# 123456jack/decision-making-and-path-planning

Hardware: AMD Instinct MI355X
Metric: planning ticks/sec (batched scenes), 512x512 grid (higher is better)
Workload: dtype f64; 1 GPU; BASELINE configs[1]: 1024 scenes/GPU, 512x512 grid, 64 static obstacles; scenes_per_gpu=1024, global_scenes=1024, grid=512, obstacles=64, parallelism=scene-sharded x1, RCCL scatter/gather outside the timed region, algorithmic_bytes_per_tick=276644

## Files before the change

### decision-making-and-path-planning_amd/csrc/kernels_s.hpp

```cpp
#pragma once
#include <type_traits>
#include "dev_geom.hpp"

#ifndef DMPP_PRIO_T2
#define DMPP_PRIO_T2 12
#define DMPP_PRIO_T3 36
#endif
namespace dmpp {

__device__ __forceinline__ uint64_t mix64(uint64_t v)
{
    uint64_t z = v + 0x9e3779b97f4a7c15ull;
    z = (z ^ (z >> 30)) * 0xbf58476d1ce4e5b9ull;
    z = (z ^ (z >> 27)) * 0x94d049bb133111ebull;
    return z ^ (z >> 31);
}

__device__ __forceinline__ int cell_of(const PlannerConfig& c, GlobalPoint2D origin, double x, double y)
{
    int ix = (int)floor((x - origin.x) / c.cell);
    int iy = (int)floor((y - origin.y) / c.cell);
    ix = clampi(ix, 0, c.grid_w - 1); iy = clampi(iy, 0, c.grid_h - 1);
    return iy * c.grid_w + ix;
}
// ... 169 lines not shown
            run = (go && stop != 0u && !((B0 >> bit) & 1u)) ? (int)((uint32_t)rr | (fP << 12) | (fM << 13)) : run;
            go = go && stop == 0u && cand != 0;
        }
    }
    return run;
}

struct Footprint { double ox, oy, R2; int ix0, ix1, iy0, iy1; };

__device__ __forceinline__ Footprint footprint_of(const PlannerConfig& c, GlobalPoint2D origin, const ObPoint& o, int W, int H)
{
    Footprint f;
    const double R = (double)o.radius + c.inflate;
    f.ox = o.x; f.oy = o.y; f.R2 = R * R;
    f.ix0 = max((int)floor((o.x - R - origin.x) / c.cell) - 1, 0);
    f.ix1 = min((int)floor((o.x + R - origin.x) / c.cell) + 1, W - 1);
    f.iy0 = max((int)floor((o.y - R - origin.y) / c.cell) - 1, 0);
    f.iy1 = min((int)floor((o.y + R - origin.y) / c.cell) + 1, H - 1);
    return f;
}

__device__ __forceinline__ bool exact_span(double ou, double org, double cell, double inv_cell, double dv2, double R2, double cq, int ic,
                                           int lo, int hi, int& a, int& b)
{
    if (dv2 > R2) return false;
    auto pred = [&](int i) { const double du = (org + ((double)i + 0.5) * cell) - ou; return du * du + dv2 <= R2; };
    const double h2 = R2 - dv2;
    const double half = __builtin_amdgcn_sqrt(h2);
    const double xa = (ou - half - org) * inv_cell - 0.5, xb = (ou + half - org) * inv_cell - 0.5;
    a = clampi((int)ceil(xa), lo - 1, hi + 1);
    b = clampi((int)floor(xb), lo - 1, hi + 1);
    {
        const double lim = 0.5 - (half * 0x1p-24 + cq) * inv_cell;
        const bool sure = (h2 >= R2 * 0x1p-40) & (fabs((xa - floor(xa)) - 0.5) < lim) & (fabs((xb - floor(xb)) - 0.5) < lim);
        if (__builtin_expect(sure, 1)) { a = max(a, lo); b = min(b, hi); return a <= b; }
    }
    asm volatile("" : "+v"(ic), "+v"(lo), "+v"(hi));
    const bool pa = pred(a), pa1 = pred(a - 1), pb = pred(b), pb1 = pred(b + 1);
    if (__builtin_expect(!((a <= b) & pa & !pa1 & pb & !pb1), 0)) {
        const bool c0 = pred(ic), c1 = pred(ic - 1), c2 = pred(ic + 1);
        if (!(c0 | c1 | c2)) return false;
        const int t = c0 ? ic : (c1 ? ic - 1 : ic + 1);
        if ((t < lo && !pred(lo)) || (t > hi && !pred(hi))) return false;
        a = clampi(min(a, t), lo - 1, hi + 1); b = clampi(max(b, t), lo - 1, hi + 1);
#pragma nounroll
        while (a >= lo && pred(a - 1)) a--;
#pragma nounroll
        while (a <= hi && !pred(a)) a++;
#pragma nounroll
        while (b <= hi && pred(b + 1)) b++;
#pragma nounroll
        while (b >= lo && b >= a && !pred(b)) b--;
    }
    a = max(a, lo); b = min(b, hi);
    return a <= b;
}

template <class F>
__device__ __forceinline__ void for_words(int p0, int p1, F&& f)
{
    for (int w = p0 >> 5; w <= (p1 >> 5); w++) {
        const int lo = max(p0 - (w << 5), 0), hi = min(p1 - (w << 5), 31);
        const uint32_t bits = (hi == 31 ? 0xFFFFFFFFu : ((2u << hi) - 1u)) & ~((1u << lo) - 1u);
        f(w, bits);
    }
}

template <int SW>
__device__ __forceinline__ int block_excl_scan(int v, int tid, int* s_wave )
{
    const int lane = tid & 63, wv = tid >> 6;
    int incl = v;
#pragma unroll
    for (int sft = 1; sft < DMPP_WAVE; sft <<= 1) { const int t = __shfl_up(incl, sft, 64); if (lane >= sft) incl += t; }
    if (lane == DMPP_WAVE - 1) s_wave[wv] = incl;
    __syncthreads();
    int base = 0, total = 0;
    for (int q = 0; q < SW; q++) { const int t = s_wave[q]; if (q < wv) base += t; total += t; }
    if (tid == 0) s_wave[SW] = total;
    __syncthreads();
    return base + incl - v;
}

template <int SW, class Emit>
__device__ __forceinline__ void for_each_span(const PlannerConfig& c, const SceneIn& si, const ObPoint* __restrict__ obs, int m, Emit&& emit)
{
    const int tid = threadIdx.x, lane = tid & 63, wv = tid >> 6;
    const int W = c.grid_w, H = c.grid_h;
    const bool colhalf = lane >= 32;
    const int l32 = lane & 31;
    const double cell = c.cell, inv_cell = 1.0 / c.cell;
    const GlobalPoint2D origin = si.grid_origin;
    const double org_u = colhalf ? origin.y : origin.x, org_v = colhalf ? origin.x : origin.y;
    const double cq_scene = 0x1p-47 * (2.0 * (fabs(origin.x) + fabs(origin.y)) + (double)max(W, H) * cell) + 0x1p-36 * cell;
    auto bcast_d = [](double v, int src) {
        const int lo = __builtin_amdgcn_readlane(__double2loint(v), src), hi = __builtin_amdgcn_readlane(__double2hiint(v), src);
        return __hiloint2double(hi, lo);
    };
    for (int base = 0; base < m; base += SW * DMPP_WAVE) {
        Footprint f; f.ox = f.oy = f.R2 = 0; f.ix0 = f.iy0 = 0; f.ix1 = f.iy1 = -1;
        int icx = 0, icy = 0;
        const int j = base + wv + SW * lane;
        if (j < m) {
            f = footprint_of(c, origin, obs[j], W, H);
            icx = (int)floor((f.ox - origin.x) / cell);
            icy = (int)floor((f.oy - origin.y) / cell);
        }
        const unsigned long long anym = wave_ballot(j < m && f.ix1 >= f.ix0 && f.iy1 >= f.iy0);
        const int left = m - base - wv;
        const int cnt = left <= 0 ? 0 : min(DMPP_WAVE, (left + SW - 1) / SW);
        for (int q = 0; q < cnt; q++) {
            if (!((anym >> q) & 1ull)) continue;
            const double fx = bcast_d(f.ox, q), fy = bcast_d(f.oy, q), R2 = bcast_d(f.R2, q);
            const int ix0 = __builtin_amdgcn_readlane(f.ix0, q), ix1 = __builtin_amdgcn_readlane(f.ix1, q);
            const int iy0 = __builtin_amdgcn_readlane(f.iy0, q), iy1 = __builtin_amdgcn_readlane(f.iy1, q);
            const int jcx = __builtin_amdgcn_readlane(icx, q), jcy = __builtin_amdgcn_readlane(icy, q);
            const double ou = colhalf ? fy : fx, ov = colhalf ? fx : fy;
            const int ic = colhalf ? jcy : jcx, l0 = colhalf ? ix0 : iy0, l1 = colhalf ? ix1 : iy1, lo = colhalf ? iy0 : ix0, hi = colhalf ? iy1 : ix1;
            const double cq = cq_scene + 0x1p-30 * (1.0 + R2);
            for (int l = l0 + l32; l <= l1; l += 32) {
                const double dv = (org_v + ((double)l + 0.5) * cell) - ov;
                int a, b;
                const bool any = exact_span(ou, org_u, cell, inv_cell, dv * dv, R2, cq, ic, lo, hi, a, b);
                if (any) emit(colhalf, l, a, b);
            }
        }
    }
}

template <int SW, class Emit>
__device__ __forceinline__ void for_each_rough_span(const PlannerConfig& c, const SceneIn& si, const ObPoint* __restrict__ obs, int m, Emit&& emit)
{
    const int tid = threadIdx.x, lane = tid & 63, wv = tid >> 6;
    const int W = c.grid_w, H = c.grid_h;
    const bool colhalf = lane >= 32;
    const int l32 = lane & 31;
    const float cellf = (float)c.cell, inv_cellf = (float)(1.0 / c.cell);
    const GlobalPoint2D origin = si.grid_origin;
    const double extent = (double)max(W, H) * c.cell;
    auto bcast_f = [](float v, int src) { return __int_as_float(__builtin_amdgcn_readlane(__float_as_int(v), src)); };
    for (int base = 0; base < m; base += SW * DMPP_WAVE) {
        float rx = 0, ry = 0, r2m = -1.0f;
        int ix0 = 0, ix1 = -1, iy0 = 0, iy1 = -1;
        const int j = base + wv + SW * lane;
        if (j < m) {
            const Footprint f = footprint_of(c, origin, obs[j], W, H);
            ix0 = f.ix0; ix1 = f.ix1; iy0 = f.iy0; iy1 = f.iy1;
            const double R = sqrt(f.R2), S = extent + R;
            rx = (float)(f.ox - origin.x); ry = (float)(f.oy - origin.y);
            r2m = (float)((f.R2 + 4.0 * (R * S * 0x1p-21 + f.R2 * 0x1p-23)) * (1.0 + 0x1p-22));
        }
        const unsigned long long anym = wave_ballot(j < m && ix1 >= ix0 && iy1 >= iy0);
        const int left = m - base - wv;
        const int cnt = left <= 0 ? 0 : min(DMPP_WAVE, (left + SW - 1) / SW);
        for (int q = 0; q < cnt; q++) {
            if (!((anym >> q) & 1ull)) continue;
            const float fx = bcast_f(rx, q), fy = bcast_f(ry, q), R2 = bcast_f(r2m, q);
            const int jx0 = __builtin_amdgcn_readlane(ix0, q), jx1 = __builtin_amdgcn_readlane(ix1, q);
            const int jy0 = __builtin_amdgcn_readlane(iy0, q), jy1 = __builtin_amdgcn_readlane(iy1, q);
            const float ou = colhalf ? fy : fx, ov = colhalf ? fx : fy;
            const int l0 = colhalf ? jx0 : jy0, l1 = colhalf ? jx1 : jy1, lo = colhalf ? jy0 : jx0, hi = colhalf ? jy1 : jx1;
            for (int l = l0 + l32; l <= l1; l += 32) {
                const float dv = ((float)l + 0.5f) * cellf - ov;
                const float h2 = R2 - dv * dv;
                if (h2 < 0.0f) continue;
                const float half = __builtin_sqrtf(h2);
                const int a = max((int)floorf((ou - half) * inv_cellf) - 2, lo), b = min((int)floorf((ou + half) * inv_cellf) + 2, hi);
                if (a <= b) emit(colhalf, l, a, b);
            }
        }
    }
}

template <int K, int SW>
__device__ __forceinline__ int build_sparse_views(const PlannerConfig& c, const SceneIn& si, const ObPoint* __restrict__ obs, int m,
                                                  const SparseView<K>& vr, const SparseView<K>& vc, int budget, int* s_wave,
                                                  long long* tmark = nullptr)
{
    using M = typename SparseView<K>::M;
    const int tid = threadIdx.x;
    const int W = c.grid_w, H = c.grid_h;
    int tm_i = 0;
    auto mark = [&]() { if (tmark) tmark[tm_i++] = clock64(); };
    mark();
    for (int l = tid; l < H; l += (SW * DMPP_WAVE)) vr.clear_line(l);
    for (int l = tid; l < W; l += (SW * DMPP_WAVE)) vc.clear_line(l);
    __syncthreads();
    mark(); mark();
    auto mark_words = [&](bool colhalf, int l, int a, int b) {
        const int wa = a >> 5, wb = b >> 5;
        const M bits = (M)((((M)2) << (wb - wa)) - (M)1) << wa;
        if (colhalf) vc.or_mask(l, bits); else vr.or_mask(l, bits);
    };
#ifdef DMPP_EXACT_PASS1
    for_each_span<SW>(c, si, obs, m, mark_words);
#else
    for_each_rough_span<SW>(c, si, obs, m, mark_words);
#endif
    __syncthreads();
    mark();
    auto place = [&](const SparseView<K>& vw) {
        const int NL = vw.NL, per = (NL + (SW * DMPP_WAVE) - 1) / (SW * DMPP_WAVE);
        const int l0 = tid * per, l1 = min(l0 + per, NL);
        int cnt = 0;
        for (int l = l0; l < l1; l++) cnt += popc_m(vw.mask_of(l));
        int off = block_excl_scan<SW>(cnt, tid, s_wave);
        const int total = s_wave[SW];
        for (int l = l0; l < l1; l++) { const int k = popc_m(vw.mask_of(l)); vw.set_off(l, (uint32_t)off); off += k; }
        __syncthreads();
        return total;
    };
    const int total_r = place(vr), total_c = place(vc);
    const int need = max(total_r, total_c);
    mark();
    if (need > budget) return need;
    for (int i = tid; i < total_r; i += (SW * DMPP_WAVE)) vr.data[i] = 0;
    for (int i = tid; i < total_c; i += (SW * DMPP_WAVE)) vc.data[i] = 0;
    __syncthreads();
    mark();
    const SparseView<K> vw = (tid & 32) ? vc : vr;
    for_each_span<SW>(c, si, obs, m, [&](bool, int l, int a, int b) {
        const LineM<M> lm = vw.line(l);
        for_words(a, b, [&](int w, uint32_t bits) {
            __hip_atomic_fetch_or(&vw.data[lm.off + popc_m((M)(lm.mask & ((((M)1) << w) - (M)1)))], bits, __ATOMIC_RELAXED, __HIP_MEMORY_SCOPE_WORKGROUP);
        });
    });
    __syncthreads();
    mark();
    return need;
}

template <int SW>
__device__ __forceinline__ void build_dense_views(const PlannerConfig& c, const SceneIn& si, const ObPoint* __restrict__ obs, int m,
                                                  uint32_t* __restrict__ bm, DMPP_LDS uint64_t* nz_row, DMPP_LDS uint64_t* nz_col)
{
    const int tid = threadIdx.x;
    const int W = c.grid_w, H = c.grid_h, WW = W >> 5, HW = H >> 5, NW = (W * H) >> 5;
    uint32_t* bmT = bm + NW;
    {
        uint4* z4 = reinterpret_cast<uint4*>(bm);
        const uint4 z = { 0u, 0u, 0u, 0u };
        for (int i = tid; i < (2 * NW) >> 2; i += (SW * DMPP_WAVE)) z4[i] = z;
    }
    __threadfence();
    __syncthreads();
    for_each_span<SW>(c, si, obs, m, [&](bool colhalf, int l, int a, int b) {
        uint32_t* line = colhalf ? bmT + (size_t)l * HW : bm + (size_t)l * WW;
        for_words(a, b, [&](int w, uint32_t bits) { atomicOr(&line[w], bits); });
    });
    __threadfence();
    __syncthreads();
    for (int v = 0; v < 2; v++) {
        const uint32_t* src = v ? bmT : bm;
        DMPP_LDS uint64_t* nz = v ? nz_col : nz_row;
        const int LW = v ? HW : WW, NL = v ? W : H;
        for (int line = tid; line < NL; line += (SW * DMPP_WAVE)) {
            uint64_t msk = 0;
            for (int w = 0; w < LW; w++) msk |= (uint64_t)min(src[line * LW + w], 1u) << w;
            nz[line] = msk;
        }
    }
    __syncthreads();
}

template <int K>
__device__ __forceinline__ void sparse_clear_cell(const SparseView<K>& vw, int line, int pos)
{
    using M = typename SparseView<K>::M;
    const LineM<M> lm = vw.line(line);
    const int w = pos >> 5;
    if (lm.mask & (((M)1) << w)) vw.data[lm.off + popc_m((M)(lm.mask & ((((M)1) << w) - (M)1)))] &= ~(1u << (pos & 31));
}

namespace rules {
constexpr int dxs(int s) { return (s == 0 || s == 1 || s == 7) ? 1 : ((s >= 3 && s <= 5) ? -1 : 0); }
constexpr int dys(int s) { return (s >= 1 && s <= 3) ? 1 : ((s >= 5) ? -1 : 0); }
constexpr int rule_code(int d, int s)
{
    const int rel = (s - d) & 7;
    const bool is_start = d == 8, d_odd = (d & 1) != 0 && !is_start, d_even = !d_odd && !is_start;
    const bool jump0 = (is_start && (s & 1) == 0) || (d_even && rel == 0) || (d_odd && (rel == 1 || rel == 7));
    const bool plain = (is_start && (s & 1) != 0) || (d_odd && rel == 0);
    const bool sided = (d_even && (rel == 1 || rel == 7)) || (d_odd && (rel == 2 || rel == 6));
    return jump0 ? 1 : (plain ? 2 : (sided ? 3 : 0));
}
constexpr int side_offset(int d, int s, bool want_y)
{
    const bool d_odd = (d & 1) != 0 && d != 8;
    const int a = want_y ? dys(s) - dys(d & 7) : dxs(s) - dxs(d & 7);
    return d_odd ? a / 2 : a;
}
constexpr uint64_t code_rows(int d0)
{
    uint64_t t = 0;
    for (int d = d0; d < d0 + 4; d++) for (int s = 0; s < 8; s++) t |= (uint64_t)rule_code(d, s) << ((d - d0) * 16 + 2 * s);
    return t;
}
constexpr uint32_t start_row() { uint32_t t = 0; for (int s = 0; s < 8; s++) t |= (uint32_t)rule_code(8, s) << (2 * s); return t; }
constexpr uint32_t kDxTab = 0x901Au, kDyTab = 0x01A9u;
constexpr bool tables_ok()
{
    for (int d = 0; d < 8; d++) if (((int)((kDxTab >> (2 * d)) & 3u) - 1) != dxs(d) || ((int)((kDyTab >> (2 * d)) & 3u) - 1) != dys(d)) return false;
    for (int d = 0; d <= 8; d++) for (int s = 0; s < 8; s++) if (rule_code(d, s) == 3) {
        const int ax = dxs(s) - dxs(d & 7), ay = dys(s) - dys(d & 7);
        if ((ax >> (d & 1)) != side_offset(d, s, false) || (ay >> (d & 1)) != side_offset(d, s, true)) return false;
    }
    return true;
}
static_assert(tables_ok(), "direction tables / side offsets");
constexpr uint64_t kCodeLo = code_rows(0), kCodeHi = code_rows(4);
constexpr uint32_t kCodeStart = start_row();
}

template <int CL>
struct SearchLds {
    static constexpr int kClosedLog = CL, kClosedTab = 1 << CL, kClosedMax = 3 << (CL - 2);
    uint32_t o_ent[kOpenCap];
    uint16_t o_f2[kOpenCap];
    uint16_t o_run[kOpenCap];
    uint32_t c_tab[kClosedTab];
    uint16_t c_info[kClosedTab];
    uint16_t c_seq[kClosedTab];
    uint32_t job[kMaxDiag + 8];
    int s_wave[kSearchSetupWavesWide + 1];
    int s_flag;
};

struct SearchOut { int status, n_exp, n_push, n_rounds, path_cost, path_len; uint64_t digest; };

template <class LDS>
__device__ __forceinline__ uint64_t hash_digest(const LDS& L, int lane)
{
    uint64_t dg = 0;
    for (int i = lane; i < LDS::kClosedTab; i += DMPP_WAVE) {
        const uint32_t e = L.c_tab[i]; const uint32_t sq = L.c_seq[i];
        if (e && sq != 0xFFFFu) dg += mix64(((uint64_t)sq << 32) | (uint64_t)(e - 1u));
    }
    return dg;
}

template <class LDS>
__device__ __forceinline__ int squeeze_open(LDS& L, int n_open, int lane)
{
    int w = 0;
    for (int q0 = 0; q0 < n_open; q0 += DMPP_WAVE) {
        const int i = q0 + lane;
        uint32_t f2 = 0xFFFFu, ee = 0; uint16_t rr = 0;
        if (i < n_open) { f2 = L.o_f2[i]; ee = L.o_ent[i]; rr = L.o_run[i]; }
        const bool alive = f2 != 0xFFFFu;
        const unsigned long long am = wave_ballot(alive);
        wave_order();
        if (alive) {
            const int r = (int)__builtin_amdgcn_mbcnt_hi((unsigned)(am >> 32), __builtin_amdgcn_mbcnt_lo((unsigned)am, 0u));
            L.o_f2[w + r] = (uint16_t)f2; L.o_ent[w + r] = ee; L.o_run[w + r] = rr;
        }
        w += __popcll(am);
        wave_order();
    }
    for (int i = w + lane; i < n_open; i += DMPP_WAVE) L.o_f2[i] = 0xFFFFu;
    wave_order();
    return w;
}

template <class LDS>
__device__ __forceinline__ int spill_open(LDS& L, int n_open , int lane, uint2* __restrict__ ospill, int& sp_n, uint32_t& sp_min)
{
    constexpr int keep = kOpenCap / 2;
    if (n_open <= keep) return n_open;
    uint32_t K[kOpenCap / DMPP_WAVE];
#pragma unroll
    for (int k = 0; k < kOpenCap / DMPP_WAVE; k++) {
        const int slot = lane + DMPP_WAVE * k;
        K[k] = slot < n_open ? (((uint32_t)L.o_f2[slot] << 16) | (0xFFFFu - (uint32_t)slot)) : 0xFFFFFFFFu;
    }
    uint32_t lo = 0u, hi = 0xFFFFFFFEu;
    for (int it = 0; it < 32 && lo < hi; it++) {
        const uint32_t mid = lo + ((hi - lo) >> 1);
        int cnt = 0;
#pragma unroll
        for (int k = 0; k < kOpenCap / DMPP_WAVE; k++) cnt += __popcll(wave_ballot(K[k] <= mid));
        if (cnt >= keep) hi = mid; else lo = mid + 1u;
    }
    uint32_t mn = 0xFFFFu;
    int base = sp_n;
#pragma unroll
    for (int k = 0; k < kOpenCap / DMPP_WAVE; k++) {
        const int slot = lane + DMPP_WAVE * k;
        const bool out = slot < n_open && K[k] > lo;
        const unsigned long long bm = wave_ballot(out);
        if (out) {
            const int r = (int)__builtin_amdgcn_mbcnt_hi((unsigned)(bm >> 32), __builtin_amdgcn_mbcnt_lo((unsigned)bm, 0u));
            const uint32_t f2 = L.o_f2[slot];
            ospill[base + r] = make_uint2(L.o_ent[slot], f2 | ((uint32_t)L.o_run[slot] << 16));
            L.o_f2[slot] = 0xFFFFu;
            mn = min(mn, f2);
        }
        base += __popcll(bm);
    }
    sp_n = base;
    sp_min = min(sp_min, wave_min_u32(mn));
// ... 461 lines not shown
            wave_sync();
            for (int i = lane; i < keep / 2; i += DMPP_WAVE) {
                const int a0 = path[i], b0 = path[keep - 1 - i];
                path[i] = b0; path[keep - 1 - i] = a0;
            }
        }
    }
    DBG_MARK(6)
    int n_push = my_pushes;
#pragma unroll
    for (int sft = 32; sft >= 1; sft >>= 1) n_push += __shfl_xor(n_push, sft, 64);
    n_push += 1;
    R.status = status; R.n_exp = n_exp; R.n_push = n_push; R.n_rounds = n_rounds; R.path_cost = path_cost; R.path_len = path_len; R.digest = digest;
    return R;
#undef DBG_MARK
}

template <class LDS>
__device__ __forceinline__ void reset_search_lds(LDS& L, int start, int goal, int W, int lane)
{
    for (int i = lane; i < LDS::kClosedTab; i += DMPP_WAVE) L.c_tab[i] = 0;
    for (int i = lane; i < kOpenCap; i += DMPP_WAVE) L.o_f2[i] = 0xFFFFu;
    wave_order();
    if (lane == 0) {
        const int sx = start % W, sy = start / W;
        L.o_ent[0] = (uint32_t)sx | ((uint32_t)sy << 12) | (8u << 24);
        L.o_f2[0] = (uint16_t)(hfun(sx, sy, goal % W, goal / W) >> 1);
        L.o_run[0] = 0;
    }
    wave_order();
}

__device__ __forceinline__ void publish_search(GridOut& go, const SearchOut& R, int start, int goal)
{
    go.order_digest = R.digest; go.status = R.status; go.n_expanded = R.n_exp; go.n_pushed = R.n_push; go.n_rounds = R.n_rounds;
    go.path_len = R.path_len; go.path_cost = R.path_cost; go.start_cell = start; go.goal_cell = goal;
}

#ifdef DMPP_DEBUG_SEARCH
__device__ __forceinline__ void publish_debug(int32_t* path, int max_path, const long long* t, const int* cn, long long t_setup, long long t_total)
{
    int32_t* dbg = path + max_path - 16;
    dbg[0] = cn[0]; dbg[1] = cn[1]; dbg[2] = cn[2]; dbg[3] = cn[3]; dbg[4] = cn[4];
    dbg[5] = (int)(t[0] >> 4); dbg[6] = (int)(t[1] >> 4); dbg[7] = (int)(t[2] >> 4); dbg[8] = (int)(t[3] >> 4); dbg[9] = (int)(t[4] >> 4);
    dbg[10] = (int)(t[6] >> 4); dbg[11] = (int)((t[0] + t[1] + t[2] + t[3] + t[4] + t[5] + t[6]) >> 4); dbg[12] = (int)(t_setup >> 4); dbg[13] = (int)(t_total >> 4);
    dbg[14] = (int)__builtin_amdgcn_s_getreg((31 << 11) | 4);
    dbg[15] = (int)__builtin_amdgcn_s_getreg((31 << 11) | 20);
    for (int i = 7; i < 16; i++) path[max_path - 64 + i] = (int)(t[i] >> 4);
}
#endif

template <int K, int SW, bool SPILL>
__device__ __forceinline__ void search_scene(const PlannerConfig& c, int scene, int w_base, int order_cap, int budget, const SceneIn* __restrict__ in,
         const ObPoint* __restrict__ obs_now, uint32_t* __restrict__ gclosed, uint16_t* __restrict__ pinfo, int32_t* __restrict__ orders,
         int32_t* __restrict__ paths, GridOut* __restrict__ gout, uint32_t* __restrict__ gbitmaps, int32_t* __restrict__ cost_out,
         int32_t* __restrict__ overflow, int32_t* __restrict__ need_max, uint2* __restrict__ ospill_all, int spill_cap,
         int32_t* __restrict__ retry_list, int32_t* __restrict__ retry_cnt,
         SearchLds<closed_log_of<K>()>& L, unsigned char* smem_raw)
{
    using LdsT = SearchLds<closed_log_of<K>()>;
    constexpr unsigned kViewsAt = 0;
    const long long t_begin = clock64();
    const int tid = threadIdx.x, lane = tid & (DMPP_WAVE - 1), wv = tid >> 6;
    const int W = c.grid_w, H = c.grid_h, N = W * H, WW = W >> 5, HW = H >> 5;
    const SceneIn& si = in[scene];
    SparseView<K> vr, vc;
    {
        DMPP_LDS unsigned char* p = (DMPP_LDS unsigned char*)smem_raw + kViewsAt;
        unsigned used = 0;
        if constexpr (K == 2) {
            vr.meta = p; vc.meta = p + (unsigned)H * 8u;
            vr.off2 = (DMPP_LDS uint16_t*)(p + (unsigned)(H + W) * 8u); vc.off2 = vr.off2 + H;
            used = (unsigned)(H + W) * 10u;
        } else {
            constexpr unsigned mb = (unsigned)sparse_meta_bytes_per_line<K>();
            vr.meta = p; vc.meta = p + (unsigned)H * mb;
            vr.off2 = nullptr; vc.off2 = nullptr;
            used = (unsigned)(H + W) * mb;
        }
        used = (used + 15u) & ~15u;
        vr.data = (DMPP_LDS uint32_t*)(p + used); vc.data = vr.data + budget;
        vr.LW = WW; vr.NL = H; vc.LW = HW; vc.NL = W;
    }
    for (int i = tid; i < LdsT::kClosedTab; i += (SW * DMPP_WAVE)) L.c_tab[i] = 0;
    for (int i = tid; i < kOpenCap; i += (SW * DMPP_WAVE)) L.o_f2[i] = 0xFFFFu;
    const ObPoint* obs = obs_now + si.obs_off;
#ifdef DMPP_DEBUG_SEARCH
    long long tmark[8] = { 0, 0, 0, 0, 0, 0, 0, 0 };
    const int need = budget > 0 ? build_sparse_views<K, SW>(c, si, obs, si.obs_n, vr, vc, budget, L.s_wave, tmark) : 1;
#else
    const int need = budget > 0 ? build_sparse_views<K, SW>(c, si, obs, si.obs_n, vr, vc, budget, L.s_wave) : 1;
#endif
    const bool dense = need > budget;
    if (tid == 0) { if (budget > 0) atomicMax(need_max, need); overflow[scene] = dense ? 1 : 0; }
    uint32_t* bm = gbitmaps + (size_t)scene * 2 * (N >> 5);
    DMPP_LDS uint64_t* nz_row = (DMPP_LDS uint64_t*)((DMPP_LDS unsigned char*)smem_raw + kViewsAt);
    DMPP_LDS uint64_t* nz_col = nz_row + H;
    if (dense) { __syncthreads(); build_dense_views<SW>(c, si, obs, si.obs_n, bm, nz_row, nz_col); }
    const DenseView dr{ bm, nz_row, WW, H }, dc{ bm + (N >> 5), nz_col, HW, W };
    const int start = cell_of(c, si.grid_origin, si.loc.globalpoint.x, si.loc.globalpoint.y);
    const int goal = cell_of(c, si.grid_origin, si.goal.x, si.goal.y);
    const bool goal_blocked = dense ? cell_blocked(dr, goal % W, goal / W) : cell_blocked(vr, goal % W, goal / W);
    __syncthreads();
    if (!goal_blocked && tid == 0) {
        const int sx = start % W, sy = start / W;
        if (dense) {
            bm[start >> 5] &= ~(1u << (start & 31));
            bm[(N >> 5) + sx * HW + (sy >> 5)] &= ~(1u << (sy & 31));
            __threadfence();
        } else {
            sparse_clear_cell(vr, sy, sx);
            sparse_clear_cell(vc, sx, sy);
        }
        L.o_ent[0] = (uint32_t)sx | ((uint32_t)sy << 12) | (8u << 24);
        L.o_f2[0] = (uint16_t)(hfun(sx, sy, goal % W, goal / W) >> 1);
        L.o_run[0] = 0;
    }
    __syncthreads();
    int32_t* path = paths + (size_t)scene * c.max_path;
    if (wv != 0) return;
    __builtin_amdgcn_s_setprio(1);
    const long long t_setup = clock64() - t_begin;
    SearchOut R; R.status = DMPP_G_GOAL_BLOCKED; R.n_exp = 0; R.n_push = 0; R.n_rounds = 0; R.path_cost = 0; R.path_len = 0; R.digest = 0;
    uint32_t* closed = gclosed + (size_t)scene * (N >> 5);
    uint16_t* pin = pinfo + (size_t)scene * N;
    int32_t* order = orders ? orders + (size_t)scene * order_cap : nullptr;
    uint2* ospill = ospill_all ? ospill_all + (size_t)scene * spill_cap : nullptr;
#ifdef DMPP_DEBUG_SEARCH
    long long dbg_t[16] = { 0, 0, 0, 0, 0, 0, 0, 0, 0, 0, 0, 0, 0, 0, 0, 0 }; int dbg_c[8] = { 0, 0, 0, 0, 0, 0, 0, 0 };
    if (!goal_blocked) R = dense ? search_core<SPILL>(c, L, dr, dc, start, goal, order_cap, closed, pin, order, path, SPILL ? ospill : nullptr, lane, dbg_t, dbg_c)
                                 : search_core<SPILL>(c, L, vr, vc, start, goal, order_cap, closed, pin, order, path, SPILL ? ospill : nullptr, lane, dbg_t, dbg_c);
    if (lane == 0) {
        publish_debug(path, c.max_path, dbg_t, dbg_c, t_setup, clock64() - t_begin);
        int32_t* d2 = path + c.max_path - 32;
        d2[0] = (int)(tmark[0] - t_begin); for (int i = 1; i < 7; i++) d2[i] = (int)(tmark[i] - tmark[i - 1]); d2[7] = (int)(t_begin + t_setup - tmark[6]);
    }
#else
    if (!goal_blocked) R = dense ? search_core<SPILL>(c, L, dr, dc, start, goal, order_cap, closed, pin, order, path, SPILL ? ospill : nullptr, lane)
                                 : search_core<SPILL>(c, L, vr, vc, start, goal, order_cap, closed, pin, order, path, SPILL ? ospill : nullptr, lane);
#endif
    if (!SPILL && __builtin_expect(R.status == DMPP_G_OVERFLOW && retry_cnt != nullptr && c.bucket_cap > kOpenCap, 0)) {
        if (lane == 0) retry_list[atomicAdd(retry_cnt, 1)] = w_base + scene;
    }
    (void)t_setup;
    if (lane == 0) {
        cost_out[scene] = (int32_t)min((clock64() - t_begin) >> kOrderShift, (long long)(kOrderClasses - 1));
        publish_search(gout[scene], R, start, goal);
    }
}

#ifdef DMPP_SEARCH_VGPR
#define DMPP_SEARCH_ATTR __attribute__((amdgpu_waves_per_eu(DMPP_SEARCH_VGPR, DMPP_SEARCH_VGPR)))
#else
#define DMPP_SEARCH_ATTR
#endif
template <int K, int SW>
__global__ void __launch_bounds__(SW * DMPP_WAVE) DMPP_SEARCH_ATTR
k_search(PlannerConfig c, int n_items, const TickGroup g, int order_cap, int budget, const int32_t* __restrict__ perm,
         uint32_t* __restrict__ gclosed, uint16_t* __restrict__ pinfo, int32_t* __restrict__ orders,
         uint32_t* __restrict__ gbitmaps, int32_t* __restrict__ cost_out,
         int32_t* __restrict__ overflow, int32_t* __restrict__ need_max, uint2* __restrict__ ospill_all, int spill_cap,
         int32_t* __restrict__ retry_list, int32_t* __restrict__ retry_cnt)
{
    extern __shared__ __align__(16) unsigned char smem_raw[];
    __shared__ SearchLds<closed_log_of<K>()> L;
    if ((int)blockIdx.x >= n_items) return;
    const int w = perm ? perm[blockIdx.x] : (int)blockIdx.x;
    if ((unsigned)w >= (unsigned)n_items) return;
    const int slot = w / g.n, scene = w - slot * g.n;
    const size_t base = (size_t)slot * g.n, N = (size_t)c.grid_w * c.grid_h;
    search_scene<K, SW, false>(c, scene, (int)base, order_cap, budget, g.in, g.obs_now + slot * g.obs_stride, gclosed + base * (N >> 5), pinfo + base * N,
                               orders ? orders + base * order_cap : nullptr, g.paths + slot * g.path_stride, g.gout + slot * g.gout_stride,
                               gbitmaps + base * 2 * (N >> 5), cost_out + base, overflow + base, need_max,
                               ospill_all ? ospill_all + base * spill_cap : nullptr, spill_cap, retry_list, retry_cnt, L, smem_raw);
}

template <int K>
__global__ void __launch_bounds__(kSearchBlock)
k_search_spill(PlannerConfig c, int n_items, const TickGroup g, int order_cap, int budget,
         uint32_t* __restrict__ gclosed, uint16_t* __restrict__ pinfo, int32_t* __restrict__ orders,
         uint32_t* __restrict__ gbitmaps, int32_t* __restrict__ cost_out,
         int32_t* __restrict__ overflow, int32_t* __restrict__ need_max, uint2* __restrict__ ospill_all, int spill_cap,
         const int32_t* __restrict__ retry_list, const int32_t* __restrict__ retry_cnt)
{
    extern __shared__ __align__(16) unsigned char smem_raw[];
    __shared__ SearchLds<closed_log_of<K>()> L;
    const int cnt = min(*retry_cnt, n_items);
    for (int i = (int)blockIdx.x; i < cnt; i += (int)gridDim.x) {
        const int w = retry_list[i];
        const int slot = w / g.n, scene = w - slot * g.n;
        const size_t base = (size_t)slot * g.n, N = (size_t)c.grid_w * c.grid_h;
        search_scene<K, kSearchSetupWaves, true>(c, scene, (int)base, order_cap, budget, g.in, g.obs_now + slot * g.obs_stride, gclosed + base * (N >> 5),
                                                 pinfo + base * N, orders ? orders + base * order_cap : nullptr, g.paths + slot * g.path_stride,
                                                 g.gout + slot * g.gout_stride, gbitmaps + base * 2 * (N >> 5), cost_out + base, overflow + base,
                                                 need_max, ospill_all ? ospill_all + base * spill_cap : nullptr, spill_cap, nullptr, nullptr, L, smem_raw);
        __syncthreads();
    }
}

template <int K>
__global__ void __launch_bounds__(kSearchBlock)
k_export_grid(PlannerConfig c, int scene, int budget, const SceneIn* __restrict__ in, const ObPoint* __restrict__ obs_now,
              uint8_t* __restrict__ out, int* __restrict__ bad)
{
    extern __shared__ __align__(16) unsigned char smem_raw[];
    __shared__ int s_wave[kSearchSetupWaves + 1];
    const int tid = threadIdx.x;
    const int W = c.grid_w, H = c.grid_h, WW = W >> 5, HW = H >> 5;
    const SceneIn& si = in[scene];
    SparseView<K> vr, vc;
    {
        DMPP_LDS unsigned char* p = (DMPP_LDS unsigned char*)smem_raw;
        unsigned used = 0;
        if constexpr (K == 2) {
            vr.meta = p; vc.meta = p + (unsigned)H * 8u;
            vr.off2 = (DMPP_LDS uint16_t*)(p + (unsigned)(H + W) * 8u); vc.off2 = vr.off2 + H;
            used = (unsigned)(H + W) * 10u;
        } else {
            constexpr unsigned mb = (unsigned)sparse_meta_bytes_per_line<K>();
            vr.meta = p; vc.meta = p + (unsigned)H * mb;
            vr.off2 = nullptr; vc.off2 = nullptr;
            used = (unsigned)(H + W) * mb;
        }
        used = (used + 15u) & ~15u;
        vr.data = (DMPP_LDS uint32_t*)(p + used); vc.data = vr.data + budget;
        vr.LW = WW; vr.NL = H; vc.LW = HW; vc.NL = W;
    }
    const ObPoint* obs = obs_now + si.obs_off;
    const int need = build_sparse_views<K, kSearchSetupWaves>(c, si, obs, si.obs_n, vr, vc, budget, s_wave);
    if (need > budget) {
        if (tid == 0) bad[1] = 1;
        for (int cell = tid; cell < W * H; cell += kSearchBlock) out[cell] = 0;
        __threadfence();
        __syncthreads();
        for_each_span<kSearchSetupWaves>(c, si, obs, si.obs_n, [&](bool colhalf, int l, int a, int b) {
            if (!colhalf) for (int x = a; x <= b; x++) out[l * W + x] = 1;
        });
        return;
    }
    int mism = 0;
    for (int cell = tid; cell < W * H; cell += kSearchBlock) {
        const int x = cell % W, y = cell / W;
        const auto mr = vr.line(y); const auto mc = vc.line(x);
        const uint32_t a = (vr.word(mr, x >> 5) >> (x & 31)) & 1u, b = (vc.word(mc, y >> 5) >> (y & 31)) & 1u;
        out[cell] = (uint8_t)a;
        mism += a != b;
    }
    if (mism) atomicAdd(&bad[0], mism);
}

}
```

Measured before the change: 5.657 million ticks/s.

## Load-balance obstacle rasterization via LDS-staged footprints and flat span work items

Replaces the per-wave obstacle broadcast loops with a block-wide scheme. Footprints for up to 128 obstacles are staged in LDS and prefix-summed into a flat list of row and column span items, which are split evenly across threads and located by binary search. The rough float pass 1 becomes an exact pass that keeps up to 12 spans per thread in registers for reuse in pass 2, and the row and column offset scans are fused into one. The staging area aliases the open list and closed set, so their initialization moves after view building; in exchange the code adds register pressure, extra barriers and a binary search per thread.

```diff
diff --git a/decision-making-and-path-planning_amd/csrc/kernels_s.hpp b/decision-making-and-path-planning_amd/csrc/kernels_s.hpp
--- a/decision-making-and-path-planning_amd/csrc/kernels_s.hpp
+++ b/decision-making-and-path-planning_amd/csrc/kernels_s.hpp
@@ -275,149 +275,250 @@
     return base + incl - v;
 }
 
+template <int SW>
+__device__ __forceinline__ void block_excl_scan2(int& v0, int& v1, int& tot0, int& tot1, int tid, int* s_wave0, int* s_wave1)
+{
+    const int lane = tid & 63, wv = tid >> 6;
+    int i0 = v0, i1 = v1;
+#pragma unroll
+    for (int sft = 1; sft < DMPP_WAVE; sft <<= 1) {
+        const int t0 = __shfl_up(i0, sft, 64), t1 = __shfl_up(i1, sft, 64);
+        if (lane >= sft) { i0 += t0; i1 += t1; }
+    }
+    if (lane == DMPP_WAVE - 1) { s_wave0[wv] = i0; s_wave1[wv] = i1; }
+    __syncthreads();
+    int b0 = 0, b1 = 0;
+    tot0 = 0; tot1 = 0;
+    for (int q = 0; q < SW; q++) {
+        const int t0 = s_wave0[q], t1 = s_wave1[q];
+        if (q < wv) { b0 += t0; b1 += t1; }
+        tot0 += t0; tot1 += t1;
+    }
+    v0 = b0 + i0 - v0; v1 = b1 + i1 - v1;
+}
+
+constexpr int kRasterChunk = 128;
+constexpr int kRasterKeep = 12;
+constexpr uint32_t kNoSpan = 0xFFFFu;
+struct RasterStage {
+    double ox[kRasterChunk], oy[kRasterChunk], R2[kRasterChunk];
+    int ix0[kRasterChunk], ix1[kRasterChunk], iy0[kRasterChunk], iy1[kRasterChunk];
+    int icx[kRasterChunk], icy[kRasterChunk];
+    int first[kRasterChunk + 1];
+};
+struct ItemRec { double ox, oy, R2; int ix0, ix1, iy0, iy1, icx, icy; };
+
+__device__ __forceinline__ ItemRec load_rec(const DMPP_LDS RasterStage* S, int j)
+{
+    ItemRec r;
+    r.ox = S->ox[j]; r.oy = S->oy[j]; r.R2 = S->R2[j];
+    r.ix0 = S->ix0[j]; r.ix1 = S->ix1[j]; r.iy0 = S->iy0[j]; r.iy1 = S->iy1[j]; r.icx = S->icx[j]; r.icy = S->icy[j];
+    return r;
+}
+
+template <int SW>
+__device__ __forceinline__ int stage_footprints(const PlannerConfig& c, const SceneIn& si, const ObPoint* __restrict__ obs, int base, int m,
+                                                DMPP_LDS RasterStage* S, int* s_wave)
+{
+    static_assert(SW * DMPP_WAVE > kRasterChunk, "one thread per staged obstacle, and one more for the total");
+    const int tid = threadIdx.x;
+    const int W = c.grid_w, H = c.grid_h;
+    const GlobalPoint2D origin = si.grid_origin;
+    const int cn = min(m - base, kRasterChunk);
+    int cnt = 0;
+    if (tid < cn) {
+        const Footprint f = footprint_of(c, origin, obs[base + tid], W, H);
+        S->ox[tid] = f.ox; S->oy[tid] = f.oy; S->R2[tid] = f.R2;
+        S->ix0[tid] = f.ix0; S->ix1[tid] = f.ix1; S->iy0[tid] = f.iy0; S->iy1[tid] = f.iy1;
+        S->icx[tid] = (int)floor((f.ox - origin.x) / c.cell);
+        S->icy[tid] = (int)floor((f.oy - origin.y) / c.cell);
+        if (f.ix1 >= f.ix0 && f.iy1 >= f.iy0) cnt = (f.iy1 - f.iy0 + 1) + (f.ix1 - f.ix0 + 1);
+    }
+    const int off = block_excl_scan<SW>(cnt, tid, s_wave);
+    if (tid <= cn) S->first[tid] = off;
+    const int total = s_wave[SW];
+    __syncthreads();
+    return total;
+}
+
+struct ItemCursor {
+    int j, fj, nx;
+    __device__ __forceinline__ void seek(const DMPP_LDS RasterStage* S, int cn, int e)
+    {
+        int lo = 0, hi = cn - 1;
+        while (lo < hi) { const int mid = (lo + hi) >> 1; if (S->first[mid + 1] > e) hi = mid; else lo = mid + 1; }
+        j = lo; fj = S->first[lo]; nx = S->first[lo + 1];
+    }
+    __device__ __forceinline__ bool step_to(const DMPP_LDS RasterStage* S, int e)
+    {
+        if (e < nx) return false;
+        do { j++; fj = nx; nx = S->first[j + 1]; } while (nx <= e);
+        return true;
+    }
+};
+
+struct SpanScene { double cell, inv_cell, cq_scene, orgx, orgy; };
+__device__ __forceinline__ SpanScene span_scene(const PlannerConfig& c, const SceneIn& si)
+{
+    SpanScene w;
+    w.cell = c.cell; w.inv_cell = 1.0 / c.cell; w.orgx = si.grid_origin.x; w.orgy = si.grid_origin.y;
+    w.cq_scene = 0x1p-47 * (2.0 * (fabs(w.orgx) + fabs(w.orgy)) + (double)max(c.grid_w, c.grid_h) * w.cell) + 0x1p-36 * w.cell;
+    return w;
+}
+
+__device__ __forceinline__ bool item_span(const SpanScene& w, const ItemRec& r, int k, bool& colhalf, int& l, int& a, int& b)
+{
+    const int nr = r.iy1 - r.iy0 + 1;
+    colhalf = k >= nr;
+    l = colhalf ? r.ix0 + (k - nr) : r.iy0 + k;
+    const double ou = colhalf ? r.oy : r.ox, ov = colhalf ? r.ox : r.oy;
+    const double org_u = colhalf ? w.orgy : w.orgx, org_v = colhalf ? w.orgx : w.orgy;
+    const int ic = colhalf ? r.icy : r.icx, lo = colhalf ? r.iy0 : r.ix0, hi = colhalf ? r.iy1 : r.ix1;
+    const double cq = w.cq_scene + 0x1p-30 * (1.0 + r.R2);
+    const double dv = (org_v + ((double)l + 0.5) * w.cell) - ov;
+    return exact_span(ou, org_u, w.cell, w.inv_cell, dv * dv, r.R2, cq, ic, lo, hi, a, b);
+}
+
 template <int SW, class Emit>
-__device__ __forceinline__ void for_each_span(const PlannerConfig& c, const SceneIn& si, const ObPoint* __restrict__ obs, int m, Emit&& emit)
-{
-    const int tid = threadIdx.x, lane = tid & 63, wv = tid >> 6;
-    const int W = c.grid_w, H = c.grid_h;
-    const bool colhalf = lane >= 32;
-    const int l32 = lane & 31;
-    const double cell = c.cell, inv_cell = 1.0 / c.cell;
-    const GlobalPoint2D origin = si.grid_origin;
-    const double org_u = colhalf ? origin.y : origin.x, org_v = colhalf ? origin.x : origin.y;
-    const double cq_scene = 0x1p-47 * (2.0 * (fabs(origin.x) + fabs(origin.y)) + (double)max(W, H) * cell) + 0x1p-36 * cell;
-    auto bcast_d = [](double v, int src) {
-        const int lo = __builtin_amdgcn_readlane(__double2loint(v), src), hi = __builtin_amdgcn_readlane(__double2hiint(v), src);
-        return __hiloint2double(hi, lo);
-    };
-    for (int base = 0; base < m; base += SW * DMPP_WAVE) {
-        Footprint f; f.ox = f.oy = f.R2 = 0; f.ix0 = f.iy0 = 0; f.ix1 = f.iy1 = -1;
-        int icx = 0, icy = 0;
-        const int j = base + wv + SW * lane;
-        if (j < m) {
-            f = footprint_of(c, origin, obs[j], W, H);
-            icx = (int)floor((f.ox - origin.x) / cell);
-            icy = (int)floor((f.oy - origin.y) / cell);
-        }
-        const unsigned long long anym = wave_ballot(j < m && f.ix1 >= f.ix0 && f.iy1 >= f.iy0);
-        const int left = m - base - wv;
-        const int cnt = left <= 0 ? 0 : min(DMPP_WAVE, (left + SW - 1) / SW);
-        for (int q = 0; q < cnt; q++) {
-            if (!((anym >> q) & 1ull)) continue;
-            const double fx = bcast_d(f.ox, q), fy = bcast_d(f.oy, q), R2 = bcast_d(f.R2, q);
-            const int ix0 = __builtin_amdgcn_readlane(f.ix0, q), ix1 = __builtin_amdgcn_readlane(f.ix1, q);
-            const int iy0 = __builtin_amdgcn_readlane(f.iy0, q), iy1 = __builtin_amdgcn_readlane(f.iy1, q);
-            const int jcx = __builtin_amdgcn_readlane(icx, q), jcy = __builtin_amdgcn_readlane(icy, q);
-            const double ou = colhalf ? fy : fx, ov = colhalf ? fx : fy;
-            const int ic = colhalf ? jcy : jcx, l0 = colhalf ? ix0 : iy0, l1 = colhalf ? ix1 : iy1, lo = colhalf ? iy0 : ix0, hi = colhalf ? iy1 : ix1;
-            const double cq = cq_scene + 0x1p-30 * (1.0 + R2);
-            for (int l = l0 + l32; l <= l1; l += 32) {
-                const double dv = (org_v + ((double)l + 0.5) * cell) - ov;
-                int a, b;
-                const bool any = exact_span(ou, org_u, cell, inv_cell, dv * dv, R2, cq, ic, lo, hi, a, b);
-                if (any) emit(colhalf, l, a, b);
-            }
-        }
-    }
-}
-
-template <int SW, class Emit>
-__device__ __forceinline__ void for_each_rough_span(const PlannerConfig& c, const SceneIn& si, const ObPoint* __restrict__ obs, int m, Emit&& emit)
-{
-    const int tid = threadIdx.x, lane = tid & 63, wv = tid >> 6;
-    const int W = c.grid_w, H = c.grid_h;
-    const bool colhalf = lane >= 32;
-    const int l32 = lane & 31;
-    const float cellf = (float)c.cell, inv_cellf = (float)(1.0 / c.cell);
-    const GlobalPoint2D origin = si.grid_origin;
-    const double extent = (double)max(W, H) * c.cell;
-    auto bcast_f = [](float v, int src) { return __int_as_float(__builtin_amdgcn_readlane(__float_as_int(v), src)); };
-    for (int base = 0; base < m; base += SW * DMPP_WAVE) {
-        float rx = 0, ry = 0, r2m = -1.0f;
-        int ix0 = 0, ix1 = -1, iy0 = 0, iy1 = -1;
-        const int j = base + wv + SW * lane;
-        if (j < m) {
-            const Footprint f = footprint_of(c, origin, obs[j], W, H);
-            ix0 = f.ix0; ix1 = f.ix1; iy0 = f.iy0; iy1 = f.iy1;
-            const double R = sqrt(f.R2), S = extent + R;
-            rx = (float)(f.ox - origin.x); ry = (float)(f.oy - origin.y);
-            r2m = (float)((f.R2 + 4.0 * (R * S * 0x1p-21 + f.R2 * 0x1p-23)) * (1.0 + 0x1p-22));
-        }
-        const unsigned long long anym = wave_ballot(j < m && ix1 >= ix0 && iy1 >= iy0);
-        const int left = m - base - wv;
-        const int cnt = left <= 0 ? 0 : min(DMPP_WAVE, (left + SW - 1) / SW);
-        for (int q = 0; q < cnt; q++) {
-            if (!((anym >> q) & 1ull)) continue;
-            const float fx = bcast_f(rx, q), fy = bcast_f(ry, q), R2 = bcast_f(r2m, q);
-            const int jx0 = __builtin_amdgcn_readlane(ix0, q), jx1 = __builtin_amdgcn_readlane(ix1, q);
-            const int jy0 = __builtin_amdgcn_readlane(iy0, q), jy1 = __builtin_amdgcn_readlane(iy1, q);
-            const float ou = colhalf ? fy : fx, ov = colhalf ? fx : fy;
-            const int l0 = colhalf ? jx0 : jy0, l1 = colhalf ? jx1 : jy1, lo = colhalf ? jy0 : jx0, hi = colhalf ? jy1 : jx1;
-            for (int l = l0 + l32; l <= l1; l += 32) {
-                const float dv = ((float)l + 0.5f) * cellf - ov;
-                const float h2 = R2 - dv * dv;
-                if (h2 < 0.0f) continue;
-                const float half = __builtin_sqrtf(h2);
-                const int a = max((int)floorf((ou - half) * inv_cellf) - 2, lo), b = min((int)floorf((ou + half) * inv_cellf) + 2, hi);
-                if (a <= b) emit(colhalf, l, a, b);
-            }
+__device__ __forceinline__ void for_each_span(const PlannerConfig& c, const SceneIn& si, const ObPoint* __restrict__ obs, int m,
+                                              DMPP_LDS RasterStage* S, int* s_wave, Emit&& emit)
+{
+    const int tid = threadIdx.x;
+    const SpanScene w = span_scene(c, si);
+    for (int base = 0; base < m; base += kRasterChunk) {
+        if (base) __syncthreads();
+        const int total = stage_footprints<SW>(c, si, obs, base, m, S, s_wave);
+        const int per = (total + SW * DMPP_WAVE - 1) / (SW * DMPP_WAVE), e0 = min(tid * per, total), e1 = min(e0 + per, total);
+        if (e0 >= e1) continue;
+        ItemCursor cu; cu.seek(S, min(m - base, kRasterChunk), e0);
+        ItemRec r = load_rec(S, cu.j);
+        for (int e = e0; e < e1; e++) {
+            if (cu.step_to(S, e)) r = load_rec(S, cu.j);
+            bool colhalf; int l, a, b;
+            if (item_span(w, r, e - cu.fj, colhalf, l, a, b)) emit(colhalf, l, a, b);
         }
     }
 }
 
 template <int K, int SW>
 __device__ __forceinline__ int build_sparse_views(const PlannerConfig& c, const SceneIn& si, const ObPoint* __restrict__ obs, int m,
-                                                  const SparseView<K>& vr, const SparseView<K>& vc, int budget, int* s_wave,
-                                                  long long* tmark = nullptr)
+                                                  const SparseView<K>& vr, const SparseView<K>& vc, int budget,
+                                                  DMPP_LDS RasterStage* S, int* s_wave, int* s_wave2, long long* tmark = nullptr)
 {
     using M = typename SparseView<K>::M;
+    constexpr int NT = SW * DMPP_WAVE;
     const int tid = threadIdx.x;
     const int W = c.grid_w, H = c.grid_h;
     int tm_i = 0;
     auto mark = [&]() { if (tmark) tmark[tm_i++] = clock64(); };
     mark();
-    for (int l = tid; l < H; l += (SW * DMPP_WAVE)) vr.clear_line(l);
-    for (int l = tid; l < W; l += (SW * DMPP_WAVE)) vc.clear_line(l);
-    __syncthreads();
-    mark(); mark();
-    auto mark_words = [&](bool colhalf, int l, int a, int b) {
-        const int wa = a >> 5, wb = b >> 5;
-        const M bits = (M)((((M)2) << (wb - wa)) - (M)1) << wa;
-        if (colhalf) vc.or_mask(l, bits); else vr.or_mask(l, bits);
-    };
-#ifdef DMPP_EXACT_PASS1
-    for_each_span<SW>(c, si, obs, m, mark_words);
-#else
-    for_each_rough_span<SW>(c, si, obs, m, mark_words);
-#endif
+    for (int l = tid; l < H; l += NT) vr.clear_line(l);
+    for (int l = tid; l < W; l += NT) vc.clear_line(l);
     __syncthreads();
     mark();
-    auto place = [&](const SparseView<K>& vw) {
-        const int NL = vw.NL, per = (NL + (SW * DMPP_WAVE) - 1) / (SW * DMPP_WAVE);
-        const int l0 = tid * per, l1 = min(l0 + per, NL);
-        int cnt = 0;
-        for (int l = l0; l < l1; l++) cnt += popc_m(vw.mask_of(l));
-        int off = block_excl_scan<SW>(cnt, tid, s_wave);
-        const int total = s_wave[SW];
-        for (int l = l0; l < l1; l++) { const int k = popc_m(vw.mask_of(l)); vw.set_off(l, (uint32_t)off); off += k; }
+    if (m <= 0) mark();
+    const SpanScene w = span_scene(c, si);
+    uint32_t keep[kRasterKeep];
+#pragma unroll
+    for (int q = 0; q < kRasterKeep; q++) keep[q] = kNoSpan;
+    auto push = [&](uint32_t v) {
+#pragma unroll
+        for (int q = 0; q + 1 < kRasterKeep; q++) keep[q] = keep[q + 1];
+        keep[kRasterKeep - 1] = v;
+    };
+    int total0 = 0;
+    for (int base = 0; base < m; base += kRasterChunk) {
+        if (base) __syncthreads();
+        const int total = stage_footprints<SW>(c, si, obs, base, m, S, s_wave);
+        if (base == 0) { total0 = total; mark(); }
+        const int per = (total + NT - 1) / NT, e0 = min(tid * per, total), e1 = min(e0 + per, total);
+        ItemCursor cu; cu.j = 0; cu.fj = 0; cu.nx = 0;
+        ItemRec r; r.ox = r.oy = r.R2 = 0; r.ix0 = r.iy0 = 0; r.ix1 = r.iy1 = -1; r.icx = r.icy = 0;
+        if (e0 < e1) { cu.seek(S, min(m - base, kRasterChunk), e0); r = load_rec(S, cu.j); }
+        for (int i = 0; i < per; i++) {
+            const int e = e0 + i;
+            uint32_t v = kNoSpan;
+            if (e < e1) {
+                if (cu.step_to(S, e)) r = load_rec(S, cu.j);
+                bool colhalf; int l, a, b;
+                if (item_span(w, r, e - cu.fj, colhalf, l, a, b)) {
+                    const int wa = a >> 5, wb = b >> 5;
+                    const M bits = (M)((((M)2) << (wb - wa)) - (M)1) << wa;
+                    const SparseView<K> vw = colhalf ? vc : vr;
+                    vw.or_mask(l, bits);
+                    v = (uint32_t)a | ((uint32_t)b << 16);
+                }
+            }
+            if (base == 0 && i < kRasterKeep) push(v);
+        }
+        if (base == 0) for (int i = per; i < kRasterKeep; i++) push(kNoSpan);
+    }
+    __syncthreads();
+    mark();
+    int total_r, total_c;
+    {
+        const int per_r = (H + NT - 1) / NT, per_c = (W + NT - 1) / NT;
+        const int r0 = min(tid * per_r, H), r1 = min(r0 + per_r, H), c0 = min(tid * per_c, W), c1 = min(c0 + per_c, W);
+        int off_r = 0, off_c = 0;
+        for (int l = r0; l < r1; l++) off_r += popc_m(vr.mask_of(l));
+        for (int l = c0; l < c1; l++) off_c += popc_m(vc.mask_of(l));
+        block_excl_scan2<SW>(off_r, off_c, total_r, total_c, tid, s_wave, s_wave2);
+        for (int l = r0; l < r1; l++) { const int k = popc_m(vr.mask_of(l)); vr.set_off(l, (uint32_t)off_r); off_r += k; }
+        for (int l = c0; l < c1; l++) { const int k = popc_m(vc.mask_of(l)); vc.set_off(l, (uint32_t)off_c); off_c += k; }
         __syncthreads();
-        return total;
-    };
-    const int total_r = place(vr), total_c = place(vc);
+    }
     const int need = max(total_r, total_c);
     mark();
     if (need > budget) return need;
-    for (int i = tid; i < total_r; i += (SW * DMPP_WAVE)) vr.data[i] = 0;
-    for (int i = tid; i < total_c; i += (SW * DMPP_WAVE)) vc.data[i] = 0;
+    for (int i = tid; i < total_r; i += NT) vr.data[i] = 0;
+    for (int i = tid; i < total_c; i += NT) vc.data[i] = 0;
     __syncthreads();
     mark();
-    const SparseView<K> vw = (tid & 32) ? vc : vr;
-    for_each_span<SW>(c, si, obs, m, [&](bool, int l, int a, int b) {
+    auto or_span = [&](bool colhalf, int l, int a, int b) {
+        const SparseView<K> vw = colhalf ? vc : vr;
         const LineM<M> lm = vw.line(l);
-        for_words(a, b, [&](int w, uint32_t bits) {
-            __hip_atomic_fetch_or(&vw.data[lm.off + popc_m((M)(lm.mask & ((((M)1) << w) - (M)1)))], bits, __ATOMIC_RELAXED, __HIP_MEMORY_SCOPE_WORKGROUP);
+        for_words(a, b, [&](int wd, uint32_t bits) {
+            __hip_atomic_fetch_or(&vw.data[lm.off + popc_m((M)(lm.mask & ((((M)1) << wd) - (M)1)))], bits, __ATOMIC_RELAXED, __HIP_MEMORY_SCOPE_WORKGROUP);
         });
-    });
+    };
+    for (int base = 0; base < m; base += kRasterChunk) {
+        int total = total0;
+        if (m > kRasterChunk) {
+            if (base) __syncthreads();
+            total = stage_footprints<SW>(c, si, obs, base, m, S, s_wave);
+        }
+        const int per = (total + NT - 1) / NT, e0 = min(tid * per, total), e1 = min(e0 + per, total);
+        const int nk = base == 0 ? min(per, kRasterKeep) : 0;
+        ItemCursor cu; cu.j = 0; cu.fj = 0; cu.nx = 0;
+        if (e0 < e1) cu.seek(S, min(m - base, kRasterChunk), e0);
+        {
+            int iy0 = 0, nr = 0, ix0 = 0;
+            bool fresh = true;
+            for (int i = 0; i < nk; i++) {
+                const uint32_t v = keep[0];
+                push(kNoSpan);
+                if (v != kNoSpan) {
+                    const int e = e0 + i;
+                    const bool moved = cu.step_to(S, e);
+                    if (moved || fresh) { iy0 = S->iy0[cu.j]; nr = S->iy1[cu.j] - iy0 + 1; ix0 = S->ix0[cu.j]; fresh = false; }
+                    const int k = e - cu.fj;
+                    const bool colhalf = k >= nr;
+                    or_span(colhalf, colhalf ? ix0 + (k - nr) : iy0 + k, (int)(v & 0xFFFFu), (int)(v >> 16));
+                }
+            }
+        }
+        ItemRec r; r.ox = r.oy = r.R2 = 0; r.ix0 = r.iy0 = 0; r.ix1 = r.iy1 = -1; r.icx = r.icy = 0;
+        bool fresh = true;
+        for (int i = nk; i < per; i++) {
+            const int e = e0 + i;
+            if (e < e1) {
+                const bool moved = cu.step_to(S, e);
+                if (moved || fresh) { r = load_rec(S, cu.j); fresh = false; }
+                bool colhalf; int l, a, b;
+                if (item_span(w, r, e - cu.fj, colhalf, l, a, b)) or_span(colhalf, l, a, b);
+            }
+        }
+    }
     __syncthreads();
     mark();
     return need;
@@ -425,7 +526,8 @@
 
 template <int SW>
 __device__ __forceinline__ void build_dense_views(const PlannerConfig& c, const SceneIn& si, const ObPoint* __restrict__ obs, int m,
-                                                  uint32_t* __restrict__ bm, DMPP_LDS uint64_t* nz_row, DMPP_LDS uint64_t* nz_col)
+                                                  uint32_t* __restrict__ bm, DMPP_LDS uint64_t* nz_row, DMPP_LDS uint64_t* nz_col,
+                                                  DMPP_LDS RasterStage* S, int* s_wave)
 {
     const int tid = threadIdx.x;
     const int W = c.grid_w, H = c.grid_h, WW = W >> 5, HW = H >> 5, NW = (W * H) >> 5;
@@ -437,7 +539,7 @@
     }
     __threadfence();
     __syncthreads();
-    for_each_span<SW>(c, si, obs, m, [&](bool colhalf, int l, int a, int b) {
+    for_each_span<SW>(c, si, obs, m, S, s_wave, [&](bool colhalf, int l, int a, int b) {
         uint32_t* line = colhalf ? bmT + (size_t)l * HW : bm + (size_t)l * WW;
         for_words(a, b, [&](int w, uint32_t bits) { atomicOr(&line[w], bits); });
     });
@@ -508,7 +610,7 @@
 template <int CL>
 struct SearchLds {
     static constexpr int kClosedLog = CL, kClosedTab = 1 << CL, kClosedMax = 3 << (CL - 2);
-    uint32_t o_ent[kOpenCap];
+    alignas(8) uint32_t o_ent[kOpenCap];
     uint16_t o_f2[kOpenCap];
     uint16_t o_run[kOpenCap];
     uint32_t c_tab[kClosedTab];
@@ -1136,21 +1238,25 @@
         vr.data = (DMPP_LDS uint32_t*)(p + used); vc.data = vr.data + budget;
         vr.LW = WW; vr.NL = H; vc.LW = HW; vc.NL = W;
     }
-    for (int i = tid; i < LdsT::kClosedTab; i += (SW * DMPP_WAVE)) L.c_tab[i] = 0;
-    for (int i = tid; i < kOpenCap; i += (SW * DMPP_WAVE)) L.o_f2[i] = 0xFFFFu;
+    static_assert(sizeof(RasterStage) <= offsetof(LdsT, job), "the staged footprints must fit the open list and the closed set");
+    DMPP_LDS RasterStage* stage = (DMPP_LDS RasterStage*)(DMPP_LDS unsigned char*)(unsigned char*)&L;
+    int* s_wave2 = (int*)L.job;
+    static_assert(sizeof(L.job) >= kSearchSetupWavesWide * sizeof(int), "second row of wave sums");
     const ObPoint* obs = obs_now + si.obs_off;
 #ifdef DMPP_DEBUG_SEARCH
     long long tmark[8] = { 0, 0, 0, 0, 0, 0, 0, 0 };
-    const int need = budget > 0 ? build_sparse_views<K, SW>(c, si, obs, si.obs_n, vr, vc, budget, L.s_wave, tmark) : 1;
+    const int need = budget > 0 ? build_sparse_views<K, SW>(c, si, obs, si.obs_n, vr, vc, budget, stage, L.s_wave, s_wave2, tmark) : 1;
 #else
-    const int need = budget > 0 ? build_sparse_views<K, SW>(c, si, obs, si.obs_n, vr, vc, budget, L.s_wave) : 1;
+    const int need = budget > 0 ? build_sparse_views<K, SW>(c, si, obs, si.obs_n, vr, vc, budget, stage, L.s_wave, s_wave2) : 1;
 #endif
     const bool dense = need > budget;
     if (tid == 0) { if (budget > 0) atomicMax(need_max, need); overflow[scene] = dense ? 1 : 0; }
     uint32_t* bm = gbitmaps + (size_t)scene * 2 * (N >> 5);
     DMPP_LDS uint64_t* nz_row = (DMPP_LDS uint64_t*)((DMPP_LDS unsigned char*)smem_raw + kViewsAt);
     DMPP_LDS uint64_t* nz_col = nz_row + H;
-    if (dense) { __syncthreads(); build_dense_views<SW>(c, si, obs, si.obs_n, bm, nz_row, nz_col); }
+    if (dense) { __syncthreads(); build_dense_views<SW>(c, si, obs, si.obs_n, bm, nz_row, nz_col, stage, L.s_wave); }
+    for (int i = tid; i < LdsT::kClosedTab; i += (SW * DMPP_WAVE)) L.c_tab[i] = 0;
+    for (int i = tid; i < kOpenCap; i += (SW * DMPP_WAVE)) L.o_f2[i] = 0xFFFFu;
     const DenseView dr{ bm, nz_row, WW, H }, dc{ bm + (N >> 5), nz_col, HW, W };
     const int start = cell_of(c, si.grid_origin, si.loc.globalpoint.x, si.loc.globalpoint.y);
     const int goal = cell_of(c, si.grid_origin, si.goal.x, si.goal.y);
@@ -1258,7 +1364,10 @@
               uint8_t* __restrict__ out, int* __restrict__ bad)
 {
     extern __shared__ __align__(16) unsigned char smem_raw[];
-    __shared__ int s_wave[kSearchSetupWaves + 1];
+    __shared__ int s_wave[kSearchSetupWaves + 1], s_wave2[kSearchSetupWaves];
+    __shared__ RasterStage stage_mem;
+    static_assert(sizeof(RasterStage) + sizeof(int) * (2 * kSearchSetupWaves + 1) <= sizeof(SearchLds<closed_log_of<0>()>), "static LDS of k_export_grid");
+    DMPP_LDS RasterStage* stage = (DMPP_LDS RasterStage*)&stage_mem;
     const int tid = threadIdx.x;
     const int W = c.grid_w, H = c.grid_h, WW = W >> 5, HW = H >> 5;
     const SceneIn& si = in[scene];
@@ -1281,13 +1390,13 @@
         vr.LW = WW; vr.NL = H; vc.LW = HW; vc.NL = W;
     }
     const ObPoint* obs = obs_now + si.obs_off;
-    const int need = build_sparse_views<K, kSearchSetupWaves>(c, si, obs, si.obs_n, vr, vc, budget, s_wave);
+    const int need = build_sparse_views<K, kSearchSetupWaves>(c, si, obs, si.obs_n, vr, vc, budget, stage, s_wave, s_wave2);
     if (need > budget) {
         if (tid == 0) bad[1] = 1;
         for (int cell = tid; cell < W * H; cell += kSearchBlock) out[cell] = 0;
         __threadfence();
         __syncthreads();
-        for_each_span<kSearchSetupWaves>(c, si, obs, si.obs_n, [&](bool colhalf, int l, int a, int b) {
+        for_each_span<kSearchSetupWaves>(c, si, obs, si.obs_n, stage, s_wave, [&](bool colhalf, int l, int a, int b) {
             if (!colhalf) for (int x = a; x <= b; x++) out[l * W + x] = 1;
         });
         return;
```

Result: faster. 5.918 million ticks/s (median of 6 runs) (+4.6%).
